# image-rs/deflate-rs

Hardware: AMD Instinct MI355X
Metric: MB/s raw input encoded (Compression::Default) + compressed size vs ref (higher is better)
Workload: dtype u8; 1 GPU; enwik8 = enwik8-like synthetic text (tests/datagen.py text_like; --enwik8 PATH takes the real file): 100000000 bytes per GPU, Compression::Default, stream-exact (P1); bytes_per_gpu=100000000, level=Compression::Default, parallelism=shard1

## Files before the change

### deflate-rs_amd/csrc/deflate_host.inc

```
#include <dlfcn.h>
#include <hsa/hsa.h>
#include <hsa/hsa_ext_amd.h>
#include <stdio.h>
#include <stdlib.h>
#include <string.h>

#include <algorithm>
#include <chrono>
#include <mutex>
#include <string>
#include <vector>

#include "../../include/mi355_deflate.h"

using namespace mi355;

extern "C" size_t mi355_deflate_bound_ex(size_t n, int wrapper, size_t hdr_len, size_t n_flush);

namespace {

struct Level {
    uint32_t count;
    uint64_t usize;
    uint16_t* X;
// ... 510 lines not shown
        return;
    }
    if (has_q)
        hipLaunchKernelGGL(k_match3<true>, dim3(ne * split), dim3(M3T), 0, st, d_in, n32, S, w.buckets, w.M, w.Mq, cfg.checks, cq,
                           aligned16, sg, ov, e_first, split, ms, mqs, sort_bad_flag(c));
    else
        hipLaunchKernelGGL(k_match3<false>, dim3(ne * split), dim3(M3T), 0, st, d_in, n32, S, w.buckets, w.M, (uint32_t*)nullptr,
                           cfg.checks, 0u, aligned16, sg, ov, e_first, split, ms, (uint32_t*)nullptr, sort_bad_flag(c));
    if (MI355_SWZ_BANKS) {
        const uint32_t units = ne * split, cus = c->n_cu ? c->n_cu : 256u;
        const uint32_t grid = (MI355_SWZ_PERSISTENT && units > cus) ? cus : units;
        if (has_q)
            hipLaunchKernelGGL(k_match3_swz<true>, dim3(grid), dim3(M3T), 0, st, d_in, n32, S, w.buckets, w.M, w.Mq, cfg.checks, cq,
                               aligned16, sg, ov, e_first, units, split, ms, mqs, sort_bad_flag(c));
        else
            hipLaunchKernelGGL(k_match3_swz<false>, dim3(grid), dim3(M3T), 0, st, d_in, n32, S, w.buckets, w.M, (uint32_t*)nullptr,
                               cfg.checks, 0u, aligned16, sg, ov, e_first, units, split, ms, (uint32_t*)nullptr, sort_bad_flag(c));
    }
}

struct SegRange {
    uint32_t seg_hi;
    Piece piece;
    const uint8_t* d_in;
    uint32_t n, pos0, n_total;
    uint32_t runup0;
    SegEnds sg;
    const uint16_t* steps;
    uint32_t* E0;
    uint32_t* xs;
    uint32_t* fixlist;
    uint32_t* n_fix;
    uint32_t* scan_part;
    uint32_t* tend;
    uint32_t* pb;
};

void launch_spec_emit(hipStream_t st, const Workspace& w, const ParseCfg& cfg, const SegRange& r) {
    const SpecFix fx{r.fixlist, w.badmap, r.n_fix};
    MI355_LAUNCH_EMIT(1, r.steps, dim3(cdiv(r.seg_hi - r.piece.seg_lo, 4)), st, r.d_in, r.n, r.seg_hi, w.M, cfg.use_quarter ? w.Mq : nullptr, cfg,
                       r.steps, r.E0, w.tokbuf, w.cnt, r.pos0, r.n_total, r.sg, r.xs, fx, r.runup0, r.piece.seg_lo);
}
void launch_spec_entries(mi355_deflate_ctx* c, hipStream_t st, const Workspace& w, const ParseCfg& cfg, const SegRange& r) {
    const uint32_t lo = r.piece.seg_lo, ns = r.seg_hi - lo;
    const SpecFix fx{r.fixlist, w.badmap, r.n_fix};
    launch_spec_emit(st, w, cfg, r);
    hipLaunchKernelGGL(k_spec_check, dim3(cdiv(ns, 256)), dim3(256), 0, st, r.seg_hi, (const uint32_t*)r.E0, (const uint32_t*)r.xs, w.badmap,
                       r.fixlist, r.n_fix, lo);
    MI355_LAUNCH_EMIT(2, r.steps, dim3(FIX_MAX / 4), st, r.d_in, r.n, r.seg_hi, w.M, cfg.use_quarter ? w.Mq : nullptr, cfg, r.steps, r.E0,
                       w.tokbuf, w.cnt, r.pos0, r.n_total, r.sg, r.xs, fx, 0u, 0u);
    hipLaunchKernelGGL(k_scan_a, dim3(cdiv(ns, 1024)), dim3(1024), 0, st, r.seg_hi, w.cnt, r.scan_part, (const uint32_t*)r.E0,
                       (const uint32_t*)r.xs, &reinterpret_cast<DevState*>(c->d_sc)->spec_bad, lo);
}
void launch_token_scan(mi355_deflate_ctx* c, hipStream_t st, const Workspace& w, const SegRange& r, bool exact) {
    const uint32_t lo = r.piece.seg_lo, ns = r.seg_hi - lo;
    if (exact)
        hipLaunchKernelGGL(k_scan_a, dim3(cdiv(ns, 1024)), dim3(1024), 0, st, r.seg_hi, w.cnt, r.scan_part, (const uint32_t*)nullptr,
                           (const uint32_t*)nullptr, (uint32_t*)nullptr, lo);
    hipLaunchKernelGGL(k_scan_b, dim3(cdiv(ns, 1024)), dim3(1024), 0, st, r.seg_hi, w.cnt, r.scan_part, w.base, c->d_sc, r.tend, r.pb, r.piece);
    hipLaunchKernelGGL(k_compact, dim3(cdiv(ns, 4)), dim3(256), 0, st, r.seg_hi, w.tokbuf, w.cnt, w.base, w.dtok, c->d_sc, lo);
}

void launch_adler(mi355_deflate_ctx* c, hipStream_t st, const uint8_t* d_in, uint64_t n) {
    const uint32_t nch = cdiv(n, ADLER_CHUNK);
    if (nch) hipLaunchKernelGGL(k_adler_part, dim3(nch), dim3(256), 0, st, d_in, (uint32_t)n, c->d_sc);
    hipLaunchKernelGGL(k_adler_fold, dim3(1), dim3(64), 0, st, (uint32_t)n, c->d_sc);
}
void launch_crc(mi355_deflate_ctx* c, hipStream_t st, const uint8_t* d_in, uint64_t n, uint32_t* part) {
    const uint32_t nch = cdiv(n, CRC_CHUNK);
    if (nch) {
        hipLaunchKernelGGL(k_crc_part, dim3(cdiv(nch, 256)), dim3(256), 0, st, d_in, (uint32_t)n, part);
        hipLaunchKernelGGL(k_crc_fold, dim3(cdiv(nch, 256)), dim3(256), 0, st, (uint32_t)n, nch, part, c->d_sc);
    }
}
int launch_frame_tail(mi355_deflate_ctx* c, hipStream_t st, const uint8_t* d_in, uint64_t n, uint32_t wrapper, const Workspace& w,
                      const uint8_t* gz_hdr, size_t gz_len, uint8_t* d_out, bool final) {
    if (wrapper == 1) {
        launch_adler(c, st, d_in, n);
        hipLaunchKernelGGL(k_zlib_frame, dim3(1), dim3(64), 0, st, c->d_sc, d_out, final ? 1u : 0u);
    }
    if (wrapper == 2) {
        HIPCHK(c, hipMemcpyAsync(w.gz_hdr, gz_hdr, gz_len, hipMemcpyHostToDevice, st));
        launch_crc(c, st, d_in, n, w.crc_part);
        hipLaunchKernelGGL(k_gzip_frame, dim3(1), dim3(64), 0, st, c->d_sc, d_out, w.gz_hdr, (uint32_t)gz_len, (uint32_t)n, final ? 1u : 0u);
    }
    return MI355_OK;
}

int launch_match_tables(mi355_deflate_ctx* c, hipStream_t st, const uint8_t* d_in, uint64_t n, Workspace& w,
                        const ParseCfg& cfg, const HashOverride& ov, bool ident, SegEnds sg, hipEvent_t ev_mid,
                        bool redo_head = false, const Arrival* arr = nullptr, uint64_t quirk_end = 0, const SortInit* init = nullptr) {
    const uint32_t n32 = (uint32_t)n;
    const int aligned16 = ((reinterpret_cast<uintptr_t>(d_in) & 15) == 0) ? 1 : 0;
    const uint32_t cq = cfg_cq(cfg);
    const bool has_q = cfg_has_q(cfg);
    if (cfg.use_quarter && cq == 0) HIPCHK(c, hipMemsetAsync(w.Mq, 0, (n + 64) * 4, st));
    const bool quirks = (ov.ns | ov.nh) != 0;
    uint32_t n_ep = (uint32_t)((n + WINDOW_SIZE - 1) / WINDOW_SIZE);
    uint32_t e_first = ident ? MI355_IDENT_EPOCHS : 0;
    if (quirks) {
        const uint64_t eq = quirk_end ? (quirk_end - 1) / WINDOW_SIZE + 2 : (uint64_t)n_ep;
        e_first = eq < n_ep ? (uint32_t)(eq > e_first ? eq : e_first) : n_ep;
    }
    const bool sorted_path = e_first < n_ep || n_ep == 0;
    uint64_t n_old = 0;
    if (e_first) {
        n_old = (uint64_t)e_first * WINDOW_SIZE + 4096;
        if (n_old > n || !sorted_path) n_old = n;
    }
    if (redo_head && sorted_path && !quirks && n_ep > e_first + 1) n_ep = e_first + 1;
    const bool piecewise = arr && arr->n > 1 && sorted_path && e_first == 0 && !redo_head;
    if (arr && arr->n > 0 && !piecewise) {
        const int rc = arrival_wait(c, st, *arr, arr->n - 1);
// ... 239 lines not shown
                    HIPCHK(c, hipStreamWaitEvent(st, c->ev_fill[1], 0));
                else
                    HIPCHK(c, hipMemsetAsync(w.levels.back().E, 0, sizeof(uint32_t), st));
                {
                    TopLevels t;
                    memset(&t, 0, sizeof t);
                    t.nl = (uint32_t)(w.levels.size() - lt);
                    if (t.nl > TOP_LEVELS) return MI355_E_ARG;
                    for (uint32_t k = 0; k < t.nl; k++) {
                        const Level& L = w.levels[lt + k];
                        t.count[k] = L.count;
                        t.usize[k] = L.usize;
                        t.X[k] = L.X;
                        t.E[k] = L.E;
                    }
                    if (lt > 0) {
                        const Level& L = w.levels[lt - 1];
                        t.count_below = L.count;
                        t.usize_below = L.usize;
                        t.X_below = L.X;
                        t.E_below = L.E;
                    }
                    hipLaunchKernelGGL(k_tree_top, dim3(1), dim3(1024), 0, st, n32, t);
                }
                for (size_t l = lt > 0 ? lt - 1 : 0; l-- > 0;) {
                    const Level& ch = w.levels[l];
                    const Level& pa = w.levels[l + 1];
                    hipLaunchKernelGGL(k_level_down, dim3(cdiv(pa.count, 64)), dim3(64), 0, st, n32, ch.count, ch.usize,
                                       ch.X, pa.count, pa.E, ch.E);
                }
                hipLaunchKernelGGL((k_emit<0, false>), dim3(cdiv(w.K0, 4)), dim3(256), 0, st, d_in, n32, w.K0, w.M, Mq, cfg, w.adv,
                                   w.levels[0].E, w.tokbuf, w.cnt, 0u, n32, sg, (uint32_t*)nullptr, SpecFix{nullptr, nullptr, nullptr}, 0u, 0u);
            } else {
                if (fill_aside) HIPCHK(c, hipStreamWaitEvent(st, c->ev_fill[1], 0));
                if (small_tail)
                    launch_spec_emit(st, w, cfg, all);
                else
                    launch_spec_entries(c, st, w, cfg, all);
            }
            if (small_tail) {
                uint32_t* const xs = spec ? w.xs : nullptr;
                if (spec && !steps)
                    hipLaunchKernelGGL((k_small_fix<true>), dim3(1), dim3(SMALL_FIX_T), 0, st, d_in, n32, w.K0, w.M, Mq, cfg, steps,
                                       w.levels[0].E, w.tokbuf, w.cnt, sg, xs, w.badmap, w.fixlist, w.nb_max, sync_tail ? 1u : 0u,
                                       &reinterpret_cast<DevState*>(c->d_sc)->spec_bad, w.base, c->d_sc, w.tend, w.pb, w.bstart, w.q13, w.tab,
                                       (pass == 0 && speculate) ? 1u : 0u);
                else
                    hipLaunchKernelGGL((k_small_fix<false>), dim3(1), dim3(SMALL_FIX_T), 0, st, d_in, n32, w.K0, w.M, Mq, cfg, steps,
                                       w.levels[0].E, w.tokbuf, w.cnt, sg, xs, w.badmap, w.fixlist, w.nb_max, sync_tail ? 1u : 0u,
                                       &reinterpret_cast<DevState*>(c->d_sc)->spec_bad, w.base, c->d_sc, w.tend, w.pb, w.bstart, w.q13, w.tab,
                                       (pass == 0 && speculate) ? 1u : 0u);
                hipLaunchKernelGGL(k_compact, dim3(cdiv(w.K0, 4)), dim3(256), 0, st, w.K0, w.tokbuf, w.cnt, w.base, w.dtok, c->d_sc, 0u);
            } else {
                launch_token_scan(c, st, w, all, !spec);
            }
        } else {
            hipLaunchKernelGGL(k_scan_zero, dim3(1), dim3(64), 0, st, c->d_sc);
        }
        if (!(m == 1 && n > 0)) {
            hipLaunchKernelGGL(k_seg_tokens, dim3(cdiv(m, 64)), dim3(64), 0, st, sg, w.K0, w.base,
                               w.levels.empty() ? nullptr : w.levels[0].E, w.tokbuf, w.cnt, c->d_sc, w.tend);
            hipLaunchKernelGGL(k_block_count, dim3(1), dim3(64), 0, st, sg, w.tend, w.pb, c->d_sc);
        }
        if (!small_tail)
            hipLaunchKernelGGL(k_block_bounds, dim3(cdiv((uint64_t)w.nb_max + 1, 4)), dim3(256), 0, st, n32, w.K0,
                               w.nb_max, cfg.mode, sg, sync_tail ? 1u : 0u, w.tend, w.pb, w.base,
                               w.levels.empty() ? nullptr : w.levels[0].E, w.tokbuf, w.dtok, c->d_sc, w.bstart, w.q13, w.tab, Piece{0u, 0u, 1u},
                               (const uint32_t*)nullptr, (pass == 0 && speculate) ? 1u : 0u);
        HIPCHK(c, mark(3));
        ev_last[pass] = 3;
        const uint32_t nbg = w.nb_max;
        const bool hist_clears = !fill_aside && small_inits;
        MI355_LAUNCH_HIST(nbg * PSPLIT, c->n_cu, st, w.dtok, c->d_sc, w.ll_freq, w.d_freq, w.tab, 0u,
                           hist_clears ? reinterpret_cast<uint32_t*>(d_out) : nullptr, (uint32_t)(need_out / 4));
        hipLaunchKernelGGL(k_block_header, dim3(nbg), dim3(128), 0, st, c->d_sc, w.ll_freq, w.d_freq, w.hdr, 0u);
        if (!fill_aside && !hist_clears) HIPCHK(c, hipMemsetAsync(d_out, 0, need_out, st));
        const bool state_with_plan = MI355_STATE_KERNEL && !zlib && !gzip;
        hipLaunchKernelGGL(k_plan, dim3(1), dim3(1024), 0, st, c->d_sc, w.hdr, w.bstart, w.q13, w.plan, bit_base,
                           (uint32_t)o->compat, w.tab.sync, reinterpret_cast<uint32_t*>(d_out), Piece{0u, 0u, 1u},
                           state_with_plan ? reinterpret_cast<uint32_t*>(c->h_sc) : (uint32_t*)nullptr);
        HIPCHK(c, mark(4));
        MI355_LAUNCH_PACK(nbg * PSPLIT, c->n_cu, st, d_in, n32, w.dtok, c->d_sc, w.hdr, w.plan, w.bstart,
                           w.q13, (uint32_t)o->compat, reinterpret_cast<uint32_t*>(d_out), w.tab, w.ll_freq, w.d_freq, 0u);
        HIPCHK(c, mark(5));
        rc = launch_frame_tail(c, st, d_in, n, o->wrapper, w, gz_hdr, gz_len, d_out, !sync_tail);
        if (rc) return rc;
        HIPCHK(c, mark(6));
        if (state_with_plan)
            ;
        else if (MI355_STATE_KERNEL)
            hipLaunchKernelGGL(k_state_out, dim3(1), dim3(64), 0, st, reinterpret_cast<const uint32_t*>(c->d_sc),
                               reinterpret_cast<uint32_t*>(c->h_sc), (uint32_t)(sizeof(DevState) / 4));
        else
            HIPCHK(c, hipMemcpyAsync(c->h_sc, c->d_sc, sizeof(DevState), hipMemcpyDeviceToHost, st));
        HIPCHK(c, hipStreamSynchronize(st));
        if (!clocks) host_ms = std::chrono::duration<float, std::milli>(std::chrono::steady_clock::now() - host_t0).count();
        HIPCHK(c, hipGetLastError());
        if (sort_order_failed(c))
            return run_encode(c, d_in, n, o, d_out, out_cap, out_len, st, ends_in, rewarm, gz_hdr, gz_len, extra);
        if (spec_entries_failed(c)) {
            c->reuse_tables = passes == 1;
            const int rc2 = run_encode(c, d_in, n, o, d_out, out_cap, out_len, st, ends_in, rewarm, gz_hdr, gz_len, extra);
            c->info.spec_fallback = c->last_spec_bad;
            return rc2;
        }

        ev_last[pass] = 6;
        if (pass == 0 && speculate) {
            bool fires;
            rc = q1_fires(c->h_sc, &fires);
            if (rc) return rc;
            if (fires) continue;
        }
        break;
    }
    const DevScalars& s = *c->h_sc;
    info.passes = passes;
    info_from_scalars(&info, s);
    c->pend_passes = passes;
    c->pend_clocks = clocks;
    if (!clocks) info.total_ms = host_ms;
    for (int p = 0; p < passes; p++) c->pend_last[p] = ev_last[p];
    if (s.ref_panic) {
        c->err = "the reference panics on this input (stored block after a buffer slide, SURVEY A.4 Q13)";
        return MI355_E_REF_PANIC;
    }
    c->last_plan = w.plan;
// ... 91 lines not shown
    const uint32_t* Mq = cfg.use_quarter ? w.Mq : nullptr;
    HIPCHK(c, hipEventRecord(c->ev_fill[0], st));
    HIPCHK(c, hipEventRecord(c->ev[0][0], st));
    if (cfg.use_quarter && cfg_cq(cfg) == 0) HIPCHK(c, hipMemsetAsync(w.Mq, 0, (n + 64) * 4, st));
    uint16_t* S = w.sorted + WINDOW_SIZE;
    const uint32_t n_ep = (uint32_t)((n + WINDOW_SIZE - 1) / WINDOW_SIZE);
    const uint32_t spe = WINDOW_SIZE / SEG;
    uint32_t e_lo = 0, seg_lo = 0;
    hipStream_t sb = two ? c->blk_stream : st;
    int np = 0;
    for (int k = 0; k < ar.n; k++) {
        const bool last = k + 1 == ar.n;
        const uint32_t e_hi = last ? n_ep : (ar.upto[k] < n_ep ? ar.upto[k] : n_ep);
        {
            const int rc = arrival_wait(c, st, ar, k);
            if (rc) return rc;
        }
        ht("arrived", k);
        if (e_hi > e_lo) {
            launch_sort(c, st, e_hi - e_lo, d_in, n32, ov, S, w.buckets, e_lo);
            if (e_lo == 0) HIPCHK(c, hipEventRecord(c->ev[0][1], st));
            launch_walk(c, st, d_in, n32, S, w, cfg, aligned16, sg, ov, e_lo, e_hi - e_lo);
            if (last) HIPCHK(c, hipEventRecord(c->ev[0][2], st));
        }
        e_lo = e_hi;
        if (k == 0) {
            HIPCHK(c, hipStreamWaitEvent(c->fill, c->ev_fill[0], 0));
            HIPCHK(c, hipMemsetAsync(c->d_sc, 0, sizeof(DevScalars), c->fill));
            HIPCHK(c, hipMemsetAsync(d_out, 0, need_out, c->fill));
            HIPCHK(c, hipEventRecord(c->ev_fill[1], c->fill));
            HIPCHK(c, hipStreamWaitEvent(sb, c->ev_fill[1], 0));
        }
        const uint32_t seg_hi = last ? w.K0 : (e_hi * spe > 64 ? (e_hi * spe - 64) / 64 * 64 : 0u);
        if (seg_hi <= seg_lo && !last) continue;
        const uint32_t p = (uint32_t)np++;
        if (sb != st) {
            HIPCHK(c, hipEventRecord(c->ev_walk[p], st));
            HIPCHK(c, hipStreamWaitEvent(sb, c->ev_walk[p], 0));
        }
        const Piece pc{seg_lo, p, last ? 1u : 0u};
        const uint32_t ns = seg_hi - seg_lo;
        if (ns) {
            const uint16_t* const steps = steps_in_emit(c, cfg, 1u) ? nullptr : w.adv;
            if (steps) hipLaunchKernelGGL(k_adv, dim3(ns), dim3(256), 0, sb, n32, w.M, Mq, cfg, w.adv, sg, seg_lo);
            const SegRange r{seg_hi, pc, d_in, n32, 0u, n32, 0u, sg, steps, w.levels[0].E, w.xs, w.fixlist + (size_t)2 * p * FIX_MAX,
                             &c->d_sc->n_fix[p], w.scan_part + seg_lo / 1024 + 2 * p, w.tend, w.pb};
            launch_spec_entries(c, sb, w, cfg, r);
            launch_token_scan(c, sb, w, r, false);
        } else {
            return MI355_OK;
        }
        const uint32_t maxb = (uint32_t)((uint64_t)ns * SEG / MAX_BUFFER_LENGTH) + 3;
        hipLaunchKernelGGL(k_block_bounds, dim3(cdiv((uint64_t)maxb + 1, 4)), dim3(256), 0, sb, n32, seg_hi, w.nb_max, cfg.mode, sg, 0u,
                           w.tend, w.pb, w.base, w.levels[0].E, w.tokbuf, w.dtok, c->d_sc, w.bstart, w.q13, w.tab, pc,
                           (const uint32_t*)(w.xs + (seg_hi - 1)), 0u);
        MI355_LAUNCH_HIST(maxb * PSPLIT, c->n_cu, sb, w.dtok, c->d_sc, w.ll_freq, w.d_freq, w.tab, p,
                           (uint32_t*)nullptr, 0u);
        hipLaunchKernelGGL(k_block_header, dim3(maxb), dim3(128), 0, sb, c->d_sc, w.ll_freq, w.d_freq, w.hdr, p);
        hipLaunchKernelGGL(k_plan, dim3(1), dim3(1024), 0, sb, c->d_sc, w.hdr, w.bstart, w.q13, w.plan, bit_base, (uint32_t)o->compat,
                           w.tab.sync, reinterpret_cast<uint32_t*>(d_out), pc, (uint32_t*)nullptr);
        HIPCHK(c, hipMemcpyAsync(c->h_piece + (size_t)p * sizeof(DevState), c->d_sc, sizeof(DevState), hipMemcpyDeviceToHost, sb));
        HIPCHK(c, hipEventRecord(c->ev_plan[p], sb));
        MI355_LAUNCH_PACK(maxb * PSPLIT, c->n_cu, sb, d_in, n32, w.dtok, c->d_sc, w.hdr, w.plan, w.bstart, w.q13,
                           (uint32_t)o->compat, reinterpret_cast<uint32_t*>(d_out), w.tab, w.ll_freq, w.d_freq, p);
        HIPCHK(c, hipEventRecord(c->ev_pack[p], sb));
        seg_lo = seg_hi;
    }
    rc = launch_frame_tail(c, sb, d_in, n, o->wrapper, w, gz_hdr, gz_len, d_out, true);
    if (rc) return rc;
    HIPCHK(c, hipMemcpyAsync(c->h_sc, c->d_sc, sizeof(DevState), hipMemcpyDeviceToHost, sb));
    bool bad = false, q1 = false;
    uint64_t sent = 0;
    hsa_agent_t a_gpu, a_cpu;
    const bool by_engine = c->engine.load() && c->engine.agents(d_out, h_out, &a_gpu, &a_cpu);
    Bounce* const by_threads = by_engine ? nullptr : bounce_for(c, h_out, out_cap);
    if (by_threads) {
        bounce_open(c);
        c->host_path |= MI355_HOST_PATH_OUT_THREADS;
    }
    ht("queued", np);
    for (int p = 0; p < np && !bad; p++) {
        HIPCHK(c, hipEventSynchronize(c->ev_plan[p]));
        ht("plan", p);
        const DevState* hs = reinterpret_cast<const DevState*>(c->h_piece + (size_t)p * sizeof(DevState));
        if (hs->spec_bad || hs->sort_bad || hs->sc.ref_panic) bad = true;
        uint64_t wpos = 0;
        if (p == 0 && hs->sc.b0_full && q1_rewarm(hs->sc.b0_last_tok, hs->sc.b0_last_pos, cfg.mode, n, &wpos)) bad = q1 = true;
        if (bad || p + 1 == np) break;
        uint64_t upto = (bit_base + hs->sc.total_bits) / 8;
        upto &= ~(uint64_t)4095;
        if (upto > sent && upto <= out_cap) {
            if (by_threads) {
                HIPCHK(c, hipEventSynchronize(c->ev_pack[p]));
                ht("pack", p);
                by_threads->out_push(h_out + sent, d_out + sent, (size_t)(upto - sent));
                c->host_path |= MI355_HOST_PATH_OUT_THREADS;
            } else if (by_engine) {
                HIPCHK(c, hipEventSynchronize(c->ev_pack[p]));
                ht("pack", p);
                if (!c->engine.start(h_out + sent, a_cpu, d_out + sent, a_gpu, (size_t)(upto - sent))) {
                    c->err = "hsa_amd_memory_async_copy failed";
                    (void)c->engine.wait_all();
                    (void)hipStreamSynchronize(st);
                    return MI355_E_HIP;
                }
            } else {
                HIPCHK(c, hipStreamWaitEvent(c->out_stream, c->ev_pack[p], 0));
// ... 937 lines not shown
```

### deflate-rs_amd/csrc/deflate_kernels.hip

```cpp
#include <hip/hip_runtime.h>
#include <stdint.h>

#include <type_traits>

#ifdef MI355_MATCH_STATS
__device__ unsigned long long g_mstats[16];
__device__ unsigned long long g_sstats[16];
#define MI355_STAT_DECL uint32_t stat_[8] = {0, 0, 0, 0, 0, 0, 0, 0};
#define MI355_STAT(i, v) stat_[i] += (v);
#define MI355_STAT_FLUSH(policy)                                                          \
    for (int i_ = 0; i_ < 8; i_++) atomicAdd(&g_mstats[i_], (unsigned long long)stat_[i_]); \
    atomicMax((policy).wgmax, stat_[0]);                                                  \
    if ((threadIdx.x & 63) == 0) {                                                        \
        unsigned long long t_ = wall_clock64();                                           \
        atomicMax((policy).wgend, t_);                                                    \
        atomicAdd((policy).wgsum, t_ - (policy).t0);                                      \
    }
#endif
#include "stages.h"

namespace mi355 {

struct GBytes {
    const uint8_t* d;
// ... 1820 lines not shown
    const uint32_t x = wave_incl_scan(v, lane);
    if (lane == 63) wtot[wv] = x;
    __syncthreads();
    uint32_t add = sc->Tcum[pc.p], all = 0;
    for (uint32_t k = 0; k < 16; k++) {
        add += red[k];
        add += k < wv ? wtot[k] : 0;
        all += wtot[k];
    }
    if (i < K) base[i] = add + x - v;
    if (tid == 0 && blockIdx.x == gridDim.x - 1) {
        uint32_t T = sc->Tcum[pc.p];
        for (uint32_t k = 0; k < 16; k++) T += red[k];
        T += all;
        const uint32_t nb = T / MAX_BUFFER_LENGTH + (pc.last ? 1u : 0u);
        sc->T = T;
        sc->nb = nb;
        sc->Tcum[pc.p + 1] = T;
        sc->nbcum[pc.p + 1] = nb;
        if (tend) {
            tend[0] = T;
            pb[0] = 0;
            pb[1] = nb;
        }
    }
}
__global__ __launch_bounds__(64) void k_state_out(const uint32_t* __restrict__ src, uint32_t* __restrict__ dst, uint32_t words) {
    for (uint32_t i = threadIdx.x; i < words; i += 64) dst[i] = src[i];
}
__global__ void k_scan_zero(DevScalars* sc) {
    if (threadIdx.x || blockIdx.x) return;
    sc->T = 0;
    sc->nb = 1;
}

__device__ __forceinline__ void k_compact_body(uint32_t bx_, uint32_t K, const uint32_t* tokbuf,
                                                 const uint32_t* cnt, const uint32_t* base,
                                                 uint32_t* dtok, const DevScalars* sc, uint32_t seg0) {
    uint64_t k = (uint64_t)bx_ * 4 + (threadIdx.x >> 6) + seg0;
    if (k >= K || spec_failed(sc)) return;
    uint32_t lane = threadIdx.x & 63;
    uint32_t c = cnt[k], b = base[k];
    const uint32_t* src = tokbuf + k * SEG;
    const uint32_t c4 = c & ~3u;
    for (uint32_t i = 4 * lane; i < c4; i += 256) *reinterpret_cast<uint4*>(dtok + b + i) = *reinterpret_cast<const uint4*>(src + i);
    if (lane < (c & 3u)) dtok[b + c4 + lane] = src[c4 + lane];
}
__global__ __launch_bounds__(256) void k_compact(uint32_t K, const uint32_t* __restrict__ tokbuf,
                                                 const uint32_t* __restrict__ cnt, const uint32_t* __restrict__ base,
                                                 uint32_t* __restrict__ dtok, const DevScalars* sc, uint32_t seg0) {
    k_compact_body(blockIdx.x, K, tokbuf, cnt, base, dtok, sc, seg0);
}

__device__ uint32_t token_start(uint32_t t, uint32_t K, const uint32_t* base, const uint32_t* E0,
                                const uint32_t* tokbuf, uint32_t lane, uint32_t* seg = nullptr) {
    uint32_t lo = 0, hi = K;
    while (hi - lo > 1) {
        const uint32_t span1 = hi - lo - 1;
        const uint32_t p = lo + 1 + (uint32_t)(((uint64_t)span1 * lane) >> 6);
        const uint32_t c = (uint32_t)__popcll(__builtin_amdgcn_ballot_w64(base[p] <= t));
        const uint32_t nlo = c ? lo + 1 + (uint32_t)(((uint64_t)span1 * (c - 1)) >> 6) : lo;
        const uint32_t nhi = c < 64 ? lo + 1 + (uint32_t)(((uint64_t)span1 * c) >> 6) : hi;
        lo = nlo;
        hi = nhi;
    }
    if (seg) *seg = lo;
    const uint32_t m = t - base[lo];
    const uint32_t* tk = tokbuf + (uint64_t)lo * SEG;
    uint32_t cov = 0;
    uint32_t tv[SEG / 64];
#pragma unroll
    for (uint32_t r = 0; r < SEG / 64; r++) tv[r] = lane + 64 * r < m ? tk[lane + 64 * r] : 0u;
#pragma unroll
    for (uint32_t r = 0; r < SEG / 64; r++) cov += lane + 64 * r < m ? tok_cover(tv[r]) : 0u;
#pragma unroll
    for (int off = 32; off; off >>= 1) cov += __shfl_xor(cov, off, 64);
    return E0[lo] + cov;
}

struct BlockTab {
    uint32_t* t0;
    uint32_t* nt;
    uint32_t* sync;
};

__global__ __launch_bounds__(64) void k_seg_tokens(SegEnds sg, uint32_t K, const uint32_t* __restrict__ base,
                                                   const uint32_t* __restrict__ E0, const uint32_t* __restrict__ tokbuf,
                                                   const uint32_t* __restrict__ cnt, const DevScalars* sc,
                                                   uint32_t* __restrict__ tend) {
    uint32_t i = blockIdx.x * 64 + threadIdx.x;
    if (i >= sg.m) return;
    uint32_t e = sg.ends[i];
    if (i + 1 == sg.m || K == 0) {
        tend[i] = sc->T;
        return;
    }
    uint32_t k = e / SEG;
    if (k >= K) {
        tend[i] = sc->T;
        return;
    }
    uint32_t pos = E0[k], c = 0, nk = cnt[k];
    const uint32_t* tk = tokbuf + (uint64_t)k * SEG;
    while (pos < e && c < nk) pos += tok_cover(tk[c++]);
    tend[i] = base[k] + c;
}

__global__ void k_block_count(SegEnds sg, const uint32_t* __restrict__ tend, uint32_t* __restrict__ pb, DevScalars* sc) {
    if (threadIdx.x || blockIdx.x) return;
    uint32_t acc = 0, prev = 0;
    for (uint32_t i = 0; i < sg.m; i++) {
        pb[i] = acc;
        acc += (tend[i] - prev) / MAX_BUFFER_LENGTH + 1;
        prev = tend[i];
    }
    pb[sg.m] = acc;
    sc->nb = acc;
}

__global__ __launch_bounds__(256) void k_block_bounds(uint32_t n, uint32_t K, uint32_t nb_max, uint32_t mode, SegEnds sg,
                                                      uint32_t sync_final, const uint32_t* __restrict__ tend,
                                                      const uint32_t* __restrict__ pb, const uint32_t* __restrict__ base,
                                                      const uint32_t* __restrict__ E0, const uint32_t* __restrict__ tokbuf,
                                                      const uint32_t* __restrict__ dtok, DevScalars* sc,
                                                      uint32_t* __restrict__ bstart, uint32_t* __restrict__ q13,
                                                      BlockTab tab, Piece pc, const uint32_t* __restrict__ xs_last, uint32_t q1_cancel) {
    const uint32_t b = sc->nbcum[pc.p] + blockIdx.x * 4 + (threadIdx.x >> 6), lane = threadIdx.x & 63;
    if (b > nb_max) return;
    const uint32_t nb = sc->nb;
    if (b > nb) return;
    if (b == nb) {
        uint32_t bs = n;
        if (!pc.last) {
            const uint32_t t = nb * (uint32_t)MAX_BUFFER_LENGTH;
            bs = t < sc->T ? token_start(t, K, base, E0, tokbuf, lane) : *xs_last;
        }
        if (lane == 0) bstart[b] = bs;
        return;
    }
    uint32_t lo = 0, hi = sg.m;
    while (hi - lo > 1) {
        uint32_t mid = lo + (hi - lo) / 2;
        if (pb[mid] <= b)
            lo = mid;
        else
            hi = mid;
    }
    const uint32_t i = lo, j = b - pb[i], nbi = pb[i + 1] - pb[i];
    const uint32_t tprev = i ? tend[i - 1] : 0;
    const uint32_t t0 = tprev + j * MAX_BUFFER_LENGTH;
    const uint32_t left = tend[i] - t0;
    const uint32_t nt = left < MAX_BUFFER_LENGTH ? left : (uint32_t)MAX_BUFFER_LENGTH;
    const uint32_t bs = nt ? token_start(t0, K, base, E0, tokbuf, lane) : sg.ends[i];
    uint32_t flag = 0;
    if (nt == MAX_BUFFER_LENGTH) {
        uint32_t t1 = t0 + MAX_BUFFER_LENGTH - 1;
        uint32_t tk = dtok[t1];
        uint32_t tp = token_start(t1, K, base, E0, tokbuf, lane);
        if (tp < WINDOW_SIZE && lane == 0) {
            sc->b0_full = 1;
            sc->b0_last_tok = tk;
            sc->b0_last_pos = tp;
            uint64_t wpos;
            if (q1_cancel && q1_rewarm(tk, tp, mode, n, &wpos)) sc->q1_cancel = 1;
        }
        if (tk >> 16) {
            uint64_t lp = (mode == MODE_LAZY) ? (uint64_t)tp + 1 : tp;
            uint64_t wdx = lp / WINDOW_SIZE;
            uint64_t wend = (wdx + 1) * (uint64_t)WINDOW_SIZE;
            uint64_t mend = (uint64_t)tp + tok_cover(tk);
            if (wdx >= 1 && mend > wend) {
                uint64_t buf_end = wdx * (uint64_t)WINDOW_SIZE + 65794;
                uint64_t have = sg.ends[i];
                if (buf_end > have) buf_end = have;
                flag = (mend + WINDOW_SIZE > buf_end) ? 2u : 1u;
            }
        }
    }
    if (lane == 0) {
        tab.t0[b] = t0;
        tab.nt[b] = nt;
        tab.sync[b] = (j + 1 == nbi && (i + 1 < sg.m || sync_final)) ? 1u : 0u;
        bstart[b] = bs;
        q13[b] = flag;
    }
}

#ifndef MI355_SMALL_TAIL
#define MI355_SMALL_TAIL 1
#endif
#ifndef MI355_SMALL_SEGS
#define MI355_SMALL_SEGS 2048
#endif
constexpr uint32_t SMALL_TAIL_SEGS = MI355_SMALL_SEGS, SMALL_FIX_T = 512, SMALL_FIX_PER = SMALL_TAIL_SEGS / SMALL_FIX_T;
template <bool STEPS>
__device__ __forceinline__ void k_small_fix_body(uint32_t bx_, const uint8_t* in, uint32_t n, uint32_t K,
                                                           const uint32_t* M, const uint32_t* Mq, ParseCfg cfg,
                                                           const uint16_t* adv, uint32_t* E0, uint32_t* tokbuf,
                                                           uint32_t* cnt, SegEnds sg, uint32_t* Xs, uint32_t* badmap, uint32_t* list,
                                                           uint32_t nb_max, uint32_t sync_final, uint32_t* spec_bad,
                                                           uint32_t* base, DevScalars* sc, uint32_t* tend,
                                                           uint32_t* pb, uint32_t* bstart,
                                                           uint32_t* q13, BlockTab tab, uint32_t q1_cancel) {
    constexpr uint32_t ROW = EmitRows<2, STEPS>::ROW, NW = SMALL_FIX_T / 64;
    __shared__ __attribute__((aligned(8))) uint16_t s_adv[NW][ROW];
    __shared__ __attribute__((aligned(8))) uint16_t s_pp[NW][ROW];
    __shared__ uint32_t s_np[NW], s_exit[NW], wtot[NW], wbad[NW], s_nfix, s_base[SMALL_TAIL_SEGS];
    const uint32_t tid = threadIdx.x, lane = tid & 63, wv = tid >> 6;
    if (Xs) {
        if (tid == 0) s_nfix = 0;
        __syncthreads();
// ... 99 lines not shown
                if (q1_cancel && q1_rewarm(tk, tp, cfg.mode, n, &wpos)) sc->q1_cancel = 1;
            }
            if (tk >> 16) {
                const uint64_t lp = (cfg.mode == MODE_LAZY) ? (uint64_t)tp + 1 : tp;
                const uint64_t wdx = lp / WINDOW_SIZE;
                const uint64_t wend = (wdx + 1) * (uint64_t)WINDOW_SIZE;
                const uint64_t mend = (uint64_t)tp + tok_cover(tk);
                if (wdx >= 1 && mend > wend) {
                    uint64_t buf_end = wdx * (uint64_t)WINDOW_SIZE + 65794;
                    const uint64_t have = sg.ends[0];
                    if (buf_end > have) buf_end = have;
                    flag = (mend + WINDOW_SIZE > buf_end) ? 2u : 1u;
                }
            }
        }
        if (lane == 0) {
            tab.t0[b] = t0;
            tab.nt[b] = nt;
            tab.sync[b] = (b + 1 == nb && sync_final) ? 1u : 0u;
            bstart[b] = bs;
            q13[b] = flag;
        }
    }
}
template <bool STEPS>
__global__ __launch_bounds__(SMALL_FIX_T) void k_small_fix(const uint8_t* __restrict__ in, uint32_t n, uint32_t K,
                                                           const uint32_t* __restrict__ M, const uint32_t* __restrict__ Mq, ParseCfg cfg,
                                                           const uint16_t* __restrict__ adv, uint32_t* E0, uint32_t* __restrict__ tokbuf,
                                                           uint32_t* cnt, SegEnds sg, uint32_t* Xs, uint32_t* badmap, uint32_t* list,
                                                           uint32_t nb_max, uint32_t sync_final, uint32_t* __restrict__ spec_bad,
                                                           uint32_t* __restrict__ base, DevScalars* sc, uint32_t* __restrict__ tend,
                                                           uint32_t* __restrict__ pb, uint32_t* __restrict__ bstart,
                                                           uint32_t* __restrict__ q13, BlockTab tab, uint32_t q1_cancel) {
    k_small_fix_body<STEPS>(blockIdx.x, in, n, K, M, Mq, cfg, adv, E0, tokbuf, cnt, sg, Xs, badmap, list, nb_max, sync_final, spec_bad, base, sc, tend, pb, bstart, q13, tab, q1_cancel);
}

__global__ __launch_bounds__(256) void k_block_table_uniform(uint64_t T2, uint32_t nb2, BlockTab tab) {
    uint32_t b = blockIdx.x * 256 + threadIdx.x;
    if (b >= nb2) return;
    uint64_t t0 = (uint64_t)b * MAX_BUFFER_LENGTH;
    uint64_t left = T2 > t0 ? T2 - t0 : 0;
    tab.t0[b] = (uint32_t)t0;
    tab.nt[b] = left < MAX_BUFFER_LENGTH ? (uint32_t)left : (uint32_t)MAX_BUFFER_LENGTH;
    tab.sync[b] = 0;
}

#ifndef MI355_PACK_SPLIT
#define MI355_PACK_SPLIT 4
#endif
constexpr uint32_t PSPLIT = MI355_PACK_SPLIT;
constexpr uint32_t PQ = MAX_BUFFER_LENGTH / PSPLIT;
static_assert(MAX_BUFFER_LENGTH % PSPLIT == 0, "parts of equal size");

template <uint32_t HT>
__device__ __forceinline__ void k_block_hist_body(uint32_t bx_, uint32_t gx_, const uint32_t* dtok, const DevScalars* sc,
                                                    uint32_t* ll_freq, uint32_t* d_freq,
                                                    BlockTab tab, uint32_t piece, uint32_t* clear, uint32_t clear_words) {
    __shared__ uint32_t h[320];
    if (clear)
        for (uint32_t i = bx_ * HT + threadIdx.x; i < clear_words; i += gx_ * HT) clear[i] = 0;
    const uint32_t b = sc->nbcum[piece] + bx_ / PSPLIT, q = bx_ % PSPLIT;
    if (b >= sc->nb || spec_failed(sc)) return;
    for (uint32_t i = threadIdx.x; i < 320; i += HT) h[i] = 0;
    __syncthreads();
    const uint32_t nt = tab.nt[b];
    const uint64_t t0 = (uint64_t)tab.t0[b] + (uint64_t)q * PQ;
    const uint64_t t1 = (uint64_t)tab.t0[b] + ((q + 1) * PQ < nt ? (q + 1) * PQ : nt);
    constexpr uint32_t HB = 8;
    for (uint64_t tb = t0 + threadIdx.x; tb < t1; tb += HT * HB) {
        uint32_t tks[HB];
#pragma unroll
        for (uint32_t k = 0; k < HB; k++) tks[k] = tb + HT * k < t1 ? dtok[tb + HT * k] : 0u;
#pragma unroll
        for (uint32_t k = 0; k < HB; k++) {
            if (tb + HT * k >= t1) break;
            const uint32_t tk = tks[k];
            if (tk >> 16) {
                uint32_t c, eb, ev;
                length_symbol(tk & 0xff, &c, &eb, &ev);
                atomicAdd(&h[257 + c], 1u);
                distance_symbol(tk >> 16, &c, &eb, &ev);
                atomicAdd(&h[288 + c], 1u);
            } else {
                atomicAdd(&h[tk & 0xff], 1u);
            }
        }
    }
    __syncthreads();
    const uint64_t slot = (uint64_t)b * PSPLIT + q;
    for (uint32_t i = threadIdx.x; i < 288; i += HT) ll_freq[slot * 288 + i] = i < NUM_LL ? h[i] : 0;
    for (uint32_t i = threadIdx.x; i < 32; i += HT) d_freq[slot * 32 + i] = i < NUM_DIST ? h[288 + i] : 0;
}
template <uint32_t HT>
__global__ __launch_bounds__(HT) void k_block_hist(const uint32_t* __restrict__ dtok, const DevScalars* sc,
                                                    uint32_t* __restrict__ ll_freq, uint32_t* __restrict__ d_freq,
                                                    BlockTab tab, uint32_t piece, uint32_t* __restrict__ clear, uint32_t clear_words) {
    k_block_hist_body<HT>(blockIdx.x, gridDim.x, dtok, sc, ll_freq, d_freq, tab, piece, clear, clear_words);
}

struct __attribute__((aligned(16))) HuffScratch {
    uint32_t key[292];
    uint32_t val[288];
    uint32_t sym[288];
    uint32_t pj[288];
    uint32_t icnt[288];
    uint32_t num[40];
};
struct HdrLds {
    uint32_t llf[288];
    uint32_t df[32];
    uint32_t clf[20];
    HuffScratch w[2];
    uint8_t ll_len[288];
    uint8_t d_len[32];
    uint8_t cl_len[20];
    uint8_t chain[320];
    uint16_t enc[320];
    uint32_t n_ll, n_d, n_enc, used;
};

#ifndef MI355_MK_WINDOW
#define MI355_MK_WINDOW 1
#endif
__device__ void mk_phase1(uint32_t* val, uint32_t n) {
    constexpr uint32_t INF = 0xFFFFFFFFu;
#if MI355_MK_WINDOW
    uint32_t root = 0, leaf = 2;
    uint32_t r0 = val[0] + val[1], r1 = INF;
    val[0] = r0;
    uint32_t l0 = leaf < n ? val[leaf] : INF, l1 = leaf + 1 < n ? val[leaf + 1] : INF;
    for (uint32_t next = 1; next + 1 < n; next++) {
        const bool t1 = r0 < l0;
        const uint32_t a = t1 ? r0 : l0;
        const uint32_t rr = t1 ? r1 : r0, ll = t1 ? l0 : l1;
        const bool t2 = rr < ll;
        const uint32_t v = a + (t2 ? rr : ll);
        const uint32_t cr = (t1 ? 1u : 0u) + (t2 ? 1u : 0u);
        if (cr >= 1) val[root] = next;
        if (cr == 2) val[root + 1] = next;
        val[next] = v;
        root += cr;
        leaf += 2 - cr;
        r0 = val[root <= next ? root : next];
        const uint32_t r1v = val[root + 1 <= next ? root + 1 : next];
        const uint32_t l0v = val[leaf < n ? leaf : n - 1], l1v = val[leaf + 1 < n ? leaf + 1 : n - 1];
        r1 = root + 1 <= next ? r1v : INF;
        l0 = leaf < n ? l0v : INF;
        l1 = leaf + 1 < n ? l1v : INF;
    }
#else
// ... 685 lines not shown
        if (nbytes & 1) r = crc_mulmod(sq, r);
        sq = crc_mulmod(sq, sq);
        nbytes >>= 1;
    }
    return r;
}

__global__ __launch_bounds__(256) void k_crc_part(const uint8_t* __restrict__ in, uint32_t n, uint32_t* __restrict__ part) {
#define BX_ blockIdx.x
#include "body_k_crc_part.inc"
#undef BX_
    const uint64_t idx = (uint64_t)blockIdx.x * 256 + tid;
    if (mylen) part[idx] = ~crc;
}

__global__ __launch_bounds__(256) void k_crc_fold(uint32_t n, uint32_t nchunks, const uint32_t* __restrict__ part,
                                                  DevScalars* sc) {
    const uint32_t i = blockIdx.x * 256 + threadIdx.x;
    uint32_t v = 0;
    if (i < nchunks) {
        const uint64_t end = (uint64_t)(i + 1) * CRC_CHUNK;
        const uint64_t after = end < n ? n - end : 0;
        v = part[i];
        if (after) v = crc_mulmod(crc_xpow8(after), v);
    }
#pragma unroll
    for (int off = 32; off; off >>= 1) v ^= __shfl_xor(v, off, 64);
    if ((threadIdx.x & 63) == 0 && v) atomicXor(&sc->crc, v);
}

__global__ void k_gzip_frame(DevScalars* sc, uint8_t* out, const uint8_t* hdr, uint32_t hdr_len, uint32_t in_len,
                             uint32_t trailer) {
#define BX_ blockIdx.x
#include "body_k_gzip_frame.inc"
#undef BX_
}

}

#define MI355_LAUNCH_EMIT(MODE, steps, grid, st, ...)                                                    \
    do {                                                                                                 \
        if (steps)                                                                                       \
            hipLaunchKernelGGL((k_emit<MODE, false>), grid, dim3(256), 0, st, __VA_ARGS__);              \
        else                                                                                             \
            hipLaunchKernelGGL((k_emit<MODE, true>), grid, dim3(256), 0, st, __VA_ARGS__);               \
    } while (0)
#define MI355_LAUNCH_HIST(units, n_cu, st, ...)                                                              \
    do {                                                                                                     \
        if ((units) <= ((n_cu) ? (n_cu) : 256u))                                                             \
            hipLaunchKernelGGL((k_block_hist<1024>), dim3(units), dim3(1024), 0, st, __VA_ARGS__);           \
        else                                                                                                 \
            hipLaunchKernelGGL((k_block_hist<256>), dim3(units), dim3(256), 0, st, __VA_ARGS__);             \
    } while (0)
#define MI355_LAUNCH_PACK(units, n_cu, st, ...)                                                              \
    do {                                                                                                     \
        if ((units) <= ((n_cu) ? (n_cu) : 256u))                                                             \
            hipLaunchKernelGGL((k_pack<PKT_SMALL>), dim3(units), dim3(PKT_SMALL), 0, st, __VA_ARGS__);       \
        else                                                                                                 \
            hipLaunchKernelGGL((k_pack<PKT_LARGE>), dim3(units), dim3(PKT_LARGE), 0, st, __VA_ARGS__);       \
    } while (0)
#include "deflate_host.inc"
#include "deflate_shard.inc"
#include "deflate_long.inc"
#include "deflate_multi.inc"
#include "deflate_batch.inc"
```

Before: 23480 MB/s.

## Fuse token compaction into the block histogram kernel on the main path

Drops the separate k_compact launch on the non-small-tail single-stream path. A new k_compact_hist kernel copies each block part's tokens from the per-segment token buffer into the dense token array while building the literal/length and distance histograms in the same pass. k_block_bounds no longer reads the dense array and instead reads the boundary token from tokbuf. The aim is to save one full read of the token stream and one kernel launch. The cost is a per-segment binary search and irregular per-segment copy loops inside the histogram kernel.

```diff
diff --git a/deflate-rs_amd/csrc/deflate_host.inc b/deflate-rs_amd/csrc/deflate_host.inc
--- a/deflate-rs_amd/csrc/deflate_host.inc
+++ b/deflate-rs_amd/csrc/deflate_host.inc
@@ -586,13 +586,13 @@
     hipLaunchKernelGGL(k_scan_a, dim3(cdiv(ns, 1024)), dim3(1024), 0, st, r.seg_hi, w.cnt, r.scan_part, (const uint32_t*)r.E0,
                        (const uint32_t*)r.xs, &reinterpret_cast<DevState*>(c->d_sc)->spec_bad, lo);
 }
-void launch_token_scan(mi355_deflate_ctx* c, hipStream_t st, const Workspace& w, const SegRange& r, bool exact) {
+void launch_token_scan(mi355_deflate_ctx* c, hipStream_t st, const Workspace& w, const SegRange& r, bool exact, bool compact = true) {
     const uint32_t lo = r.piece.seg_lo, ns = r.seg_hi - lo;
     if (exact)
         hipLaunchKernelGGL(k_scan_a, dim3(cdiv(ns, 1024)), dim3(1024), 0, st, r.seg_hi, w.cnt, r.scan_part, (const uint32_t*)nullptr,
                            (const uint32_t*)nullptr, (uint32_t*)nullptr, lo);
     hipLaunchKernelGGL(k_scan_b, dim3(cdiv(ns, 1024)), dim3(1024), 0, st, r.seg_hi, w.cnt, r.scan_part, w.base, c->d_sc, r.tend, r.pb, r.piece);
-    hipLaunchKernelGGL(k_compact, dim3(cdiv(ns, 4)), dim3(256), 0, st, r.seg_hi, w.tokbuf, w.cnt, w.base, w.dtok, c->d_sc, lo);
+    if (compact) hipLaunchKernelGGL(k_compact, dim3(cdiv(ns, 4)), dim3(256), 0, st, r.seg_hi, w.tokbuf, w.cnt, w.base, w.dtok, c->d_sc, lo);
 }
 
 void launch_adler(mi355_deflate_ctx* c, hipStream_t st, const uint8_t* d_in, uint64_t n) {
@@ -938,7 +938,7 @@
                                        (pass == 0 && speculate) ? 1u : 0u);
                 hipLaunchKernelGGL(k_compact, dim3(cdiv(w.K0, 4)), dim3(256), 0, st, w.K0, w.tokbuf, w.cnt, w.base, w.dtok, c->d_sc, 0u);
             } else {
-                launch_token_scan(c, st, w, all, !spec);
+                launch_token_scan(c, st, w, all, !spec, false);
             }
         } else {
             hipLaunchKernelGGL(k_scan_zero, dim3(1), dim3(64), 0, st, c->d_sc);
@@ -951,14 +951,18 @@
         if (!small_tail)
             hipLaunchKernelGGL(k_block_bounds, dim3(cdiv((uint64_t)w.nb_max + 1, 4)), dim3(256), 0, st, n32, w.K0,
                                w.nb_max, cfg.mode, sg, sync_tail ? 1u : 0u, w.tend, w.pb, w.base,
-                               w.levels.empty() ? nullptr : w.levels[0].E, w.tokbuf, w.dtok, c->d_sc, w.bstart, w.q13, w.tab, Piece{0u, 0u, 1u},
+                               w.levels.empty() ? nullptr : w.levels[0].E, w.tokbuf, c->d_sc, w.bstart, w.q13, w.tab, Piece{0u, 0u, 1u},
                                (const uint32_t*)nullptr, (pass == 0 && speculate) ? 1u : 0u);
         HIPCHK(c, mark(3));
         ev_last[pass] = 3;
         const uint32_t nbg = w.nb_max;
         const bool hist_clears = !fill_aside && small_inits;
-        MI355_LAUNCH_HIST(nbg * PSPLIT, c->n_cu, st, w.dtok, c->d_sc, w.ll_freq, w.d_freq, w.tab, 0u,
-                           hist_clears ? reinterpret_cast<uint32_t*>(d_out) : nullptr, (uint32_t)(need_out / 4));
+        if (small_tail)
+            MI355_LAUNCH_HIST(nbg * PSPLIT, c->n_cu, st, w.dtok, c->d_sc, w.ll_freq, w.d_freq, w.tab, 0u,
+                               hist_clears ? reinterpret_cast<uint32_t*>(d_out) : nullptr, (uint32_t)(need_out / 4));
+        else
+            MI355_LAUNCH_COMPACT_HIST(nbg * PSPLIT, c->n_cu, st, w.K0, w.tokbuf, w.cnt, w.base, w.dtok, c->d_sc, w.ll_freq, w.d_freq, w.tab,
+                                       hist_clears ? reinterpret_cast<uint32_t*>(d_out) : nullptr, (uint32_t)(need_out / 4));
         hipLaunchKernelGGL(k_block_header, dim3(nbg), dim3(128), 0, st, c->d_sc, w.ll_freq, w.d_freq, w.hdr, 0u);
         if (!fill_aside && !hist_clears) HIPCHK(c, hipMemsetAsync(d_out, 0, need_out, st));
         const bool state_with_plan = MI355_STATE_KERNEL && !zlib && !gzip;
@@ -1156,7 +1160,7 @@
         }
         const uint32_t maxb = (uint32_t)((uint64_t)ns * SEG / MAX_BUFFER_LENGTH) + 3;
         hipLaunchKernelGGL(k_block_bounds, dim3(cdiv((uint64_t)maxb + 1, 4)), dim3(256), 0, sb, n32, seg_hi, w.nb_max, cfg.mode, sg, 0u,
-                           w.tend, w.pb, w.base, w.levels[0].E, w.tokbuf, w.dtok, c->d_sc, w.bstart, w.q13, w.tab, pc,
+                           w.tend, w.pb, w.base, w.levels[0].E, w.tokbuf, c->d_sc, w.bstart, w.q13, w.tab, pc,
                            (const uint32_t*)(w.xs + (seg_hi - 1)), 0u);
         MI355_LAUNCH_HIST(maxb * PSPLIT, c->n_cu, sb, w.dtok, c->d_sc, w.ll_freq, w.d_freq, w.tab, p,
                            (uint32_t*)nullptr, 0u);
diff --git a/deflate-rs_amd/csrc/deflate_kernels.hip b/deflate-rs_amd/csrc/deflate_kernels.hip
--- a/deflate-rs_amd/csrc/deflate_kernels.hip
+++ b/deflate-rs_amd/csrc/deflate_kernels.hip
@@ -1896,8 +1896,7 @@
     k_compact_body(blockIdx.x, K, tokbuf, cnt, base, dtok, sc, seg0);
 }
 
-__device__ uint32_t token_start(uint32_t t, uint32_t K, const uint32_t* base, const uint32_t* E0,
-                                const uint32_t* tokbuf, uint32_t lane, uint32_t* seg = nullptr) {
+__device__ __forceinline__ uint32_t token_segment(uint32_t t, uint32_t K, const uint32_t* base, uint32_t lane) {
     uint32_t lo = 0, hi = K;
     while (hi - lo > 1) {
         const uint32_t span1 = hi - lo - 1;
@@ -1908,6 +1907,11 @@
         lo = nlo;
         hi = nhi;
     }
+    return lo;
+}
+__device__ uint32_t token_start(uint32_t t, uint32_t K, const uint32_t* base, const uint32_t* E0,
+                                const uint32_t* tokbuf, uint32_t lane, uint32_t* seg = nullptr) {
+    const uint32_t lo = token_segment(t, K, base, lane);
     if (seg) *seg = lo;
     const uint32_t m = t - base[lo];
     const uint32_t* tk = tokbuf + (uint64_t)lo * SEG;
@@ -1966,7 +1970,7 @@
                                                       uint32_t sync_final, const uint32_t* __restrict__ tend,
                                                       const uint32_t* __restrict__ pb, const uint32_t* __restrict__ base,
                                                       const uint32_t* __restrict__ E0, const uint32_t* __restrict__ tokbuf,
-                                                      const uint32_t* __restrict__ dtok, DevScalars* sc,
+                                                      DevScalars* sc,
                                                       uint32_t* __restrict__ bstart, uint32_t* __restrict__ q13,
                                                       BlockTab tab, Piece pc, const uint32_t* __restrict__ xs_last, uint32_t q1_cancel) {
     const uint32_t b = sc->nbcum[pc.p] + blockIdx.x * 4 + (threadIdx.x >> 6), lane = threadIdx.x & 63;
@@ -1998,9 +2002,9 @@
     const uint32_t bs = nt ? token_start(t0, K, base, E0, tokbuf, lane) : sg.ends[i];
     uint32_t flag = 0;
     if (nt == MAX_BUFFER_LENGTH) {
-        uint32_t t1 = t0 + MAX_BUFFER_LENGTH - 1;
-        uint32_t tk = dtok[t1];
-        uint32_t tp = token_start(t1, K, base, E0, tokbuf, lane);
+        uint32_t t1 = t0 + MAX_BUFFER_LENGTH - 1, sg1;
+        uint32_t tp = token_start(t1, K, base, E0, tokbuf, lane, &sg1);
+        uint32_t tk = tokbuf[(uint64_t)sg1 * SEG + (t1 - base[sg1])];
         if (tp < WINDOW_SIZE && lane == 0) {
             sc->b0_full = 1;
             sc->b0_last_tok = tk;
@@ -2206,6 +2210,17 @@
 constexpr uint32_t PQ = MAX_BUFFER_LENGTH / PSPLIT;
 static_assert(MAX_BUFFER_LENGTH % PSPLIT == 0, "parts of equal size");
 
+__device__ __forceinline__ void hist_token(uint32_t* h, uint32_t tk) {
+    if (tk >> 16) {
+        uint32_t c, eb, ev;
+        length_symbol(tk & 0xff, &c, &eb, &ev);
+        atomicAdd(&h[257 + c], 1u);
+        distance_symbol(tk >> 16, &c, &eb, &ev);
+        atomicAdd(&h[288 + c], 1u);
+    } else {
+        atomicAdd(&h[tk & 0xff], 1u);
+    }
+}
 template <uint32_t HT>
 __device__ __forceinline__ void k_block_hist_body(uint32_t bx_, uint32_t gx_, const uint32_t* dtok, const DevScalars* sc,
                                                     uint32_t* ll_freq, uint32_t* d_freq,
@@ -2228,16 +2243,7 @@
 #pragma unroll
         for (uint32_t k = 0; k < HB; k++) {
             if (tb + HT * k >= t1) break;
-            const uint32_t tk = tks[k];
-            if (tk >> 16) {
-                uint32_t c, eb, ev;
-                length_symbol(tk & 0xff, &c, &eb, &ev);
-                atomicAdd(&h[257 + c], 1u);
-                distance_symbol(tk >> 16, &c, &eb, &ev);
-                atomicAdd(&h[288 + c], 1u);
-            } else {
-                atomicAdd(&h[tk & 0xff], 1u);
-            }
+            hist_token(h, tks[k]);
         }
     }
     __syncthreads();
@@ -2250,6 +2256,90 @@
                                                     uint32_t* __restrict__ ll_freq, uint32_t* __restrict__ d_freq,
                                                     BlockTab tab, uint32_t piece, uint32_t* __restrict__ clear, uint32_t clear_words) {
     k_block_hist_body<HT>(blockIdx.x, gridDim.x, dtok, sc, ll_freq, d_freq, tab, piece, clear, clear_words);
+}
+
+#ifndef MI355_CH_UNROLL
+#define MI355_CH_UNROLL 4
+#endif
+#ifndef MI355_CH_SEGS
+#define MI355_CH_SEGS 8
+#endif
+template <uint32_t HT>
+__global__ __launch_bounds__(HT) void k_compact_hist(uint32_t K, const uint32_t* __restrict__ tokbuf, const uint32_t* __restrict__ cnt,
+                                                      const uint32_t* __restrict__ base, uint32_t* __restrict__ dtok,
+                                                      const DevScalars* sc, uint32_t* __restrict__ ll_freq,
+                                                      uint32_t* __restrict__ d_freq, BlockTab tab, uint32_t* __restrict__ clear,
+                                                      uint32_t clear_words) {
+    __shared__ uint32_t h[320], s_seg[2];
+    constexpr uint32_t NW = HT / 64;
+    const uint32_t tid = threadIdx.x, lane = tid & 63, wv = tid >> 6;
+    if (clear)
+        for (uint32_t i = blockIdx.x * HT + tid; i < clear_words; i += gridDim.x * HT) clear[i] = 0;
+    const uint32_t b = blockIdx.x / PSPLIT, q = blockIdx.x % PSPLIT;
+    if (b >= sc->nb || spec_failed(sc)) return;
+    for (uint32_t i = tid; i < 320; i += HT) h[i] = 0;
+    const uint32_t nt = tab.nt[b], bt0 = tab.t0[b];
+    const uint32_t t0 = bt0 + q * PQ, t1 = bt0 + ((q + 1) * PQ < nt ? (q + 1) * PQ : nt);
+    if (t0 < t1 && wv < 2) {
+        const uint32_t k = token_segment(wv ? t1 - 1 : t0, K, base, lane);
+        if (lane == 0) s_seg[wv] = k;
+    }
+    __syncthreads();
+    if (t0 < t1) {
+        const uint32_t k0 = s_seg[0], k1 = s_seg[1] + 1, ns = k1 - k0;
+        const uint32_t lg = ns <= MI355_CH_SEGS * NW ? 6u : (ns <= 8 * MI355_CH_SEGS * NW ? 4u : 2u);
+        const uint32_t G = 1u << lg, S = 64u >> lg, sub = lane & (G - 1), ws = lane >> lg;
+        constexpr uint32_t U = MI355_CH_UNROLL;
+        uint32_t kn = k0 + wv * S + ws, bkn = 0, cn = 0;
+        if (kn < k1) {
+            bkn = base[kn];
+            cn = cnt[kn];
+        }
+        for (uint32_t kk = k0 + wv * S; kk < k1; kk += NW * S) {
+            const uint32_t k = kk + ws, bk = bkn, c = cn;
+            kn = k + NW * S;
+            if (kn < k1) {
+                bkn = base[kn];
+                cn = cnt[kn];
+            }
+            uint32_t lo = 0, hi = 0;
+            if (k < k1) {
+                lo = t0 > bk ? t0 - bk : 0u;
+                hi = t1 - bk < c ? t1 - bk : c;
+            }
+            const uint32_t* src = tokbuf + (uint64_t)k * SEG;
+            uint32_t* dst = dtok + bk;
+            for (uint32_t i0 = (lo & ~3u) + 4 * sub; i0 < hi; i0 += 4 * G * U) {
+                uint4 v[U];
+#pragma unroll
+                for (uint32_t u = 0; u < U; u++) {
+                    const uint32_t i = i0 + 4 * G * u;
+                    v[u] = (i >= lo && i + 4 <= hi) ? *reinterpret_cast<const uint4*>(src + i) : make_uint4(0u, 0u, 0u, 0u);
+                }
+#pragma unroll
+                for (uint32_t u = 0; u < U; u++) {
+                    const uint32_t i = i0 + 4 * G * u;
+                    if (i >= lo && i + 4 <= hi) {
+                        *reinterpret_cast<uint4*>(dst + i) = v[u];
+                        hist_token(h, v[u].x);
+                        hist_token(h, v[u].y);
+                        hist_token(h, v[u].z);
+                        hist_token(h, v[u].w);
+                    } else {
+                        for (uint32_t j = i < lo ? lo : i; j < i + 4 && j < hi; j++) {
+                            const uint32_t tk = src[j];
+                            dst[j] = tk;
+                            hist_token(h, tk);
+                        }
+                    }
+                }
+            }
+        }
+    }
+    __syncthreads();
+    const uint64_t slot = (uint64_t)b * PSPLIT + q;
+    for (uint32_t i = tid; i < 288; i += HT) ll_freq[slot * 288 + i] = i < NUM_LL ? h[i] : 0;
+    for (uint32_t i = tid; i < 32; i += HT) d_freq[slot * 32 + i] = i < NUM_DIST ? h[288 + i] : 0;
 }
 
 struct __attribute__((aligned(16))) HuffScratch {
@@ -3041,6 +3131,13 @@
         else                                                                                                 \
             hipLaunchKernelGGL((k_block_hist<256>), dim3(units), dim3(256), 0, st, __VA_ARGS__);             \
     } while (0)
+#define MI355_LAUNCH_COMPACT_HIST(units, n_cu, st, ...)                                                      \
+    do {                                                                                                     \
+        if ((units) <= ((n_cu) ? (n_cu) : 256u))                                                             \
+            hipLaunchKernelGGL((k_compact_hist<1024>), dim3(units), dim3(1024), 0, st, __VA_ARGS__);         \
+        else                                                                                                 \
+            hipLaunchKernelGGL((k_compact_hist<256>), dim3(units), dim3(256), 0, st, __VA_ARGS__);           \
+    } while (0)
 #define MI355_LAUNCH_PACK(units, n_cu, st, ...)                                                              \
     do {                                                                                                     \
         if ((units) <= ((n_cu) ? (n_cu) : 256u))                                                             \
```

Result: no change. 23380 MB/s, median of 2 (-0.5%).
